# donahowe/TheaterGen

Measured on AMD Instinct MI355X. Metric: 512px 50-step char images/sec (node), CMIGBench 4-turn story, higher is better.
Workload: dtype bf16

## Files before the change

### theatergen_amd/build.py

```python
import hashlib
import os
import subprocess
import sys
from concurrent.futures import ThreadPoolExecutor

HERE = os.path.dirname(os.path.abspath(__file__))
CSRC = os.path.join(HERE, "csrc")
OBJ = os.path.join(CSRC, "_build")
LIBDIR = os.path.join(HERE, "lib")
LIB = os.path.join(LIBDIR, "libtheatergen_hip.so")
HEADER = os.path.join(os.path.dirname(HERE), "include", "theatergen_hip.h")
ARCH = "gfx950"
FLAGS = ["--offload-arch=" + ARCH, "-O3", "-std=c++17", "-fPIC",
         "-Wno-unused-result"]


EXTRA_FLAGS = {"tg_rowchain.hip": ["-mllvm", "-pragma-unroll-threshold=1000000"]}

BUILD_INFO = os.path.join(LIBDIR, "build_info.json")


def _write_build_info():
    import json

    def git(*a):
        try:
            return subprocess.run(["git", "-C", HERE] + list(a), capture_output=True, text=True).stdout.strip()
        except OSError:
            return ""
    info = {"commit": git("rev-parse", "--short", "HEAD"), "csrc_dirty": bool(git("status", "--porcelain", "--", CSRC, HEADER)),
            "sources_sha256": _digest(sources() + sorted(os.path.join(CSRC, f) for f in os.listdir(CSRC) if f.endswith(".h")) + [HEADER])[:16]}
    with open(BUILD_INFO, "w") as f:
        json.dump(info, f)


def _hipcc():
    for c in (os.environ.get("HIPCC"), "/opt/rocm/bin/hipcc", "hipcc"):
        if c and (os.path.isabs(c) and os.path.exists(c) or not os.path.isabs(c)):
            return c
    return "hipcc"


def _digest(paths):
    h = hashlib.sha256()
    for p in paths:
        with open(p, "rb") as f:
            h.update(f.read())
    h.update(" ".join(FLAGS).encode())
    for p_ in paths:
        h.update(" ".join(EXTRA_FLAGS.get(os.path.basename(p_), [])).encode())
    return h.hexdigest()


def sources():
    return sorted(os.path.join(CSRC, f) for f in os.listdir(CSRC) if f.endswith(".hip"))


def build(force=False, verbose=True, check_gate=False):
    os.makedirs(OBJ, exist_ok=True)
    os.makedirs(LIBDIR, exist_ok=True)
    srcs = sources()
    deps = [os.path.join(CSRC, f) for f in os.listdir(CSRC) if f.endswith(".h")] + [HEADER]
    hipcc = _hipcc()
    todo = []
    objs = []
    for s in srcs:
        o = os.path.join(OBJ, os.path.basename(s)[:-4] + ".o")
        stamp = o + ".sha"
        dg = _digest([s] + deps)
        objs.append(o)
        if force or not os.path.exists(o) or not os.path.exists(o + ".res") or not os.path.exists(stamp) or open(stamp).read() != dg:
            todo.append((s, o, stamp, dg))

    def compile_one(job):
        s, o, stamp, dg = job
        cmd = [hipcc] + FLAGS + EXTRA_FLAGS.get(os.path.basename(s), []) + ["-Rpass-analysis=kernel-resource-usage", "-c", s, "-o", o]
        if verbose:
            print("[build]", " ".join(cmd), flush=True)
        r = subprocess.run(cmd, capture_output=True, text=True)
        if r.returncode != 0:
            raise RuntimeError(f"hipcc failed for {s}:\n{r.stdout}\n{r.stderr}")
        with open(o + ".res", "w") as f:
            f.write(r.stderr)
        with open(stamp, "w") as f:
            f.write(dg)

    if todo:
        with ThreadPoolExecutor(max_workers=min(8, len(todo))) as ex:
            list(ex.map(compile_one, todo))
    if todo or not os.path.exists(LIB):
        cmd = [hipcc, "--offload-arch=" + ARCH, "-shared", "-fPIC", "-o", LIB] + objs
        if verbose:
            print("[build]", " ".join(cmd), flush=True)
        r = subprocess.run(cmd, capture_output=True, text=True)
        if r.returncode != 0:
            raise RuntimeError(f"link failed:\n{r.stdout}\n{r.stderr}")
    if todo or not os.path.exists(BUILD_INFO):
        _write_build_info()
    if check_gate or os.environ.get("TG_BUILD_GATE") == "1":
        write_resources(check=True, verbose=verbose, report=False)
    return LIB


RESOURCES_JSON = os.path.join(os.path.dirname(HERE), "profiles", "r6_kernel_resources.json")
HOT_GATES = [
    ("attention_kernel<bf16,48,64,true,true,false,false>", 0, 128),
    ("attention_kernel<f16,48,64,true,true,false,false>", 0, 128),
    ("attention_kernel<", 0, 256),
    ("gemm_glds_kernel<", 0, 256),
    ("conv_halo_kernel<", 0, 256),
    ("conv_slab_kernel<", 320, 256),
    ("bt_gemm_kernel<", 132, 256),
    ("rc_xattn_kernel<", 0, 256),
    ("rc_ff_kernel<", 0, 256),
    ("rc_front_kernel<", 0, 216),
    ("rc_linear_kernel<", 0, 256),
    ("skinny_gemm_kernel<", 0, 256),
    ("attn_bwd_kernel<", 0, 224),
    ("pp_gemm_kernel<bf16,2,", 0, 256),
    ("pp_gemm_kernel<f16,2,", 0, 256),
    ("pp_gemm_kernel<bf16,0,0>", 0, 256),
    ("pp_gemm_kernel<f16,0,0>", 0, 256),
    ("pp_gemm_kernel<", 256, 256),
    ("conv_in_mfma_kernel<", 0, 256),
    ("conv_out_mfma_kernel<", 0, 128),
]


def _pretty(sym):
    import re
    m = re.match(r"_ZN12_GLOBAL__N_1(\d+)", sym) or re.match(r"_Z(\d+)", sym)
    if not m:
        return sym
    n = int(m.group(1))
    base, rest = sym[m.end():m.end() + n], sym[m.end() + n:]
    if not rest.startswith("I"):
        return base
    args, i = [], 1
    while i < len(rest) and rest[i] != "E":
        if rest.startswith("DF16b", i):
            args.append("bf16"); i += 5
        elif rest.startswith("DF16_", i):
            args.append("f16"); i += 5
        elif rest[i] == "L":
            j = rest.index("E", i)
            tok = rest[i + 1:j]
            if tok[0] == "b":
                args.append("true" if tok[1:] == "1" else "false")
            else:
                args.append(re.sub(r"^[a-z]n?", lambda mm: "-" if mm.group(0).endswith("n") and len(mm.group(0)) > 1 else "", tok))
            i = j + 1
        elif rest[i] in "fidjlmb":
            args.append({"f": "float", "i": "int", "d": "double", "j": "unsigned", "l": "long", "m": "unsigned long", "b": "bool"}[rest[i]]); i += 1
        else:
            args.append("?" + rest[i:i + 12]); break
    return base + "<" + ",".join(args) + ">"


def _demangle(names):
    return [_pretty(n) for n in names]


def kernel_resources(verbose=True):
    import re
    keys = {"VGPRs": "vgprs", "AGPRs": "agprs", "ScratchSize [bytes/lane]": "scratch", "Occupancy [waves/SIMD]": "occupancy",
            "SGPRs Spill": "sgpr_spill", "VGPRs Spill": "vgpr_spill", "SGPRs": "sgprs"}
    all_recs = []
    for src in sources():
        path = os.path.join(OBJ, os.path.basename(src)[:-4] + ".o.res")
        if not os.path.exists(path):
            raise RuntimeError(f"{path} is missing: run build() first")
        cur = None
        for line in open(path).read().splitlines():
            m = re.search(r"remark: Function Name: (\S+)", line)
            if m:
                cur = {"symbol": m.group(1), "file": os.path.basename(src)}
                all_recs.append(cur)
                continue
            m = re.search(r"remark:\s+([A-Za-z][A-Za-z \[\]/]*): (\d+)", line)
            if m and cur is not None and m.group(1).strip() in keys:
                cur[keys[m.group(1).strip()]] = int(m.group(2))
    names = _demangle([r["symbol"] for r in all_recs])
    out = {}
    for r, n in zip(all_recs, names):
        r = dict(r)
        if n in out:
            n = n + " " + r["symbol"]
        out[n] = r
    if verbose:
        print(f"[resources] {len(out)} kernels", flush=True)
    return out


def check_resources(res):
    bad = []
    hits = [0] * len(HOT_GATES)
    for name, r in res.items():
        for gi, (sub, max_scratch, max_vgpr) in enumerate(HOT_GATES):
            if sub in name:
                hits[gi] += 1
                if r.get("scratch", 0) > max_scratch or r.get("vgprs", 0) > max_vgpr:
                    bad.append(f"{name}: {r.get('vgprs')} VGPRs (<= {max_vgpr}), scratch {r.get('scratch')} B (<= {max_scratch})")
                break
    for (sub, _, _), n in zip(HOT_GATES, hits):
        if n == 0:
            bad.append(f"gate '{sub}' matches no kernel")
    return bad


ASM_MFMA_KERNELS = {"tg_conv_slab_pp.o": "conv_slab_pp_kernel"}


def check_mfma_loops(verbose=True):
    import re
    import tempfile
    llvm = os.path.join(os.path.dirname(os.path.realpath(_hipcc())), "..", "lib", "llvm", "bin")
    if not os.path.exists(os.path.join(llvm, "llvm-objdump")):
        llvm = "/opt/rocm/lib/llvm/bin"
    bad = []

    def regs(tok):
        m = re.match(r"v\[(\d+):(\d+)\]", tok)
        if m:
            return set(range(int(m.group(1)), int(m.group(2)) + 1))
        m = re.match(r"v(\d+)$", tok)
        return {int(m.group(1))} if m else set()

    for obj, sub in ASM_MFMA_KERNELS.items():
        o = os.path.join(OBJ, obj)
        if not os.path.exists(o):
            continue
        with tempfile.TemporaryDirectory(prefix="tg_isa_") as td:
            fb, co = os.path.join(td, "k.fatbin"), os.path.join(td, "k.co")
            subprocess.run([os.path.join(llvm, "llvm-objcopy"), "--dump-section", ".hip_fatbin=" + fb, o], check=True)
            subprocess.run([os.path.join(llvm, "clang-offload-bundler"), "--unbundle", "--type=o", "--input=" + fb,
                            "--targets=hipv4-amdgcn-amd-amdhsa--" + ARCH, "--output=" + co], check=True)
            dis = subprocess.run([os.path.join(llvm, "llvm-objdump"), "-d", "--no-show-raw-insn", co], capture_output=True, text=True, check=True).stdout
        kern, body, kernels = None, [], []
        for line in dis.split("\n"):
            m = re.match(r"^[0-9a-f]+ <(.*)>:$", line)
            if m:
                if kern is not None:
                    kernels.append((kern, body))
                kern, body = m.group(1), []
            elif kern is not None:
                body.append(line.split("//")[0].strip())
        if kern is not None:
            kernels.append((kern, body))
        seen = 0
        for name, body in kernels:
            if sub not in name:
                continue
            mf = [i for i, t in enumerate(body) if t.startswith("v_mfma")]
            if not mf:
                continue
            seen += 1
            loop = body[mf[0]:mf[-1] + 1]
            accs = set()
            for t in loop:
                if t.startswith("v_mfma"):
                    accs |= regs(t.split(None, 1)[1].split(",")[0].strip())
            hits = [t for t in loop if t and not t.startswith("v_mfma") and any(regs(x) & accs for x in re.findall(r"v\[\d+:\d+\]|v\d+", t))]
            if hits:
                bad.append(f"{_pretty(name)}: {len(hits)} instruction(s) inside the inline-asm MFMA loop touch an accumulator register, e.g. `{hits[0]}`")
        if verbose:
            print(f"[mfma-loops] {obj}: {seen} kernels checked", flush=True)
        if seen == 0:
            bad.append(f"{obj}: no kernel matching {sub!r} with MFMAs found (the check would be vacuous)")
    return bad


def write_resources(check=False, verbose=True, report=True):
    import json
    res = kernel_resources(verbose=verbose)
    if report:
        try:
            commit = subprocess.run(["git", "rev-parse", "--short", "HEAD"], capture_output=True, text=True, cwd=HERE).stdout.strip()
        except OSError:
# ... 23 lines not shown
```

### theatergen_amd/csrc/tg_gemm.hip

```cpp
#include "tg_gemm_common.h"
#include "tg_gemm_glds.h"

namespace {

struct TileCfg { int bm, bn, bk; };
const TileCfg kTiles[] = {{128, 128, 64}, {64, 64, 64}, {128, 64, 64}, {64, 128, 64}, {128, 128, 64}, {256, 256, 64}, {128, 128, 32},
                          {128, 160, 64}, {128, 160, 64}, {128, 160, 64}};
constexpr int kNumTiles = 10;

struct Plan { int tile; bool halo; int full, tail, s, kps; long tiles_m, tiles_n; };



template <typename T>
__global__ void splitk_reduce_kernel(GemmParams p);

inline int64_t plan_workspace_bytes(const Plan& pl) {
  return pl.s > 1 ? (int64_t)pl.tail * pl.s * kTiles[pl.tile].bm * kTiles[pl.tile].bn * 4 : 0;
}

template <typename T>
int launch_reduce(const GemmParams& p, const Plan& pl, hipStream_t st) {
  if (pl.s > 1) {
    hipLaunchKernelGGL(splitk_reduce_kernel<T>, dim3((unsigned)pl.tail * 8), dim3(256), 0, st, p);
    TG_LAUNCH_CHECK();
  }
  return TG_OK;
}

inline bool halo_eligible(const tg_gemm_desc* d) {
  if (d->mode != 1 || d->stride != 1 || d->pad_mode != 0 || d->force_tile != 0 || d->force_split_k > 1 || d->act != TG_ACT_NONE || d->geglu) return false;
  if (d->c0 % BK != 0 || (d->a1 && d->c1 % BK != 0) || d->M % 128 != 0) return false;
  if (d->out_w == 8) return d->out_h == 8 && !d->upsample && d->M >= 1024;
  if (d->out_w != 16 && d->out_w != 32 && d->out_w != 64) return false;
  const int th = 128 / d->out_w;
  if (d->out_h % th != 0) return false;
  return d->M >= 4096;
}

template <typename T>
__global__ __launch_bounds__(256) void splitk_reduce_kernel(GemmParams p) {
  const int t = blockIdx.x >> 3, slice = blockIdx.x & 7;
  const int lbid = p.full_tiles + t;
  const long m0 = (long)(lbid / p.tiles_n) * p.tile_bm, n0 = (long)(lbid % p.tiles_n) * p.tile_bn;
  const int q4 = p.tile_bn / 4;
  const int rows = p.tile_bm / 8;
  const long tile_elems = (long)p.tile_bm * p.tile_bn;
  const float* base = p.ws + (long)t * p.tail_s * tile_elems;
  for (int q = threadIdx.x; q < rows * q4; q += blockDim.x) {
    const int lr = slice * rows + q / q4, lc = (q % q4) * 4;
    f32x4 s = {0.f, 0.f, 0.f, 0.f};
    for (int z = 0; z < p.tail_s; ++z) s += *reinterpret_cast<const f32x4*>(base + z * tile_elems + (long)lr * p.tile_bn + lc);
    const long m = p.patch_pwl > 0 ? patch_token(p, lbid / p.tiles_n, lr) : m0 + lr;
    epilogue_store4<T>(p, m, n0 + lc, s[0], s[1], s[2], s[3]);
  }
}


inline bool halo_eligible(const tg_gemm_desc* d);

inline long t64_max_tiles() {
  const char* e = getenv("TG_T64_MAX");
  return e ? strtol(e, nullptr, 0) : 128;
}

inline int t160_mode() {
  const char* e = getenv("TG_T160");
  return e ? (int)strtol(e, nullptr, 0) : 7;
}

inline long t3_max_tiles() {
  const char* e = getenv("TG_T3_MAX");
  return e ? strtol(e, nullptr, 0) : 256;
}

Plan make_plan(const tg_gemm_desc* d) {
  const long M = d->M, N = d->N, K = d->K;
  const bool halo = halo_eligible(d);
  int t = 0;
  if (!halo) {
    if (N <= 64 && M > 64) t = 2;
    else if (M <= 64 && N > 64) t = 3;
    else if (M <= 64 && N <= 64) t = 1;
    else if (d->mode == 0 && !d->geglu && ((M + 127) / 128) * ((N + 127) / 128) <= t64_max_tiles()) t = 1;
    else if (d->mode == 0 && !d->geglu && N <= 1280 && ((M + 127) / 128) * ((N + 127) / 128) <= t3_max_tiles()) t = 2;
    {
      const char* mk = getenv("TG_T7_MAXK");
      const long maxk = mk ? strtol(mk, nullptr, 0) : 640;
      if (t == 0 && d->mode == 0 && !d->geglu && K <= maxk && K % 32 == 0) t = 6;
      {
        const long t128 = ((M + 127) / 128) * ((N + 127) / 128);
        const char* fit = getenv("TG_T7_FIT");
        if (fit && fit[0] == '1' && t == 0 && d->mode == 0 && !d->geglu && K % 32 == 0 && t128 > 512 && t128 <= 768) t = 6;
      }
    }
    if ((t == 0 || t == 6) && d->mode == 0 && !d->geglu && d->act == TG_ACT_NONE && d->n_split <= 0 && N % 160 == 0 && M % 128 == 0 && K % 64 == 0 && (t160_mode() & 5)) {
      const long t128 = ((M + 127) / 128) * ((N + 127) / 128), s128 = (t == 6) ? 768 : 512;
      const long t160 = (M / 128) * (N / 160);
      const double eff128 = (double)t128 / (double)(((t128 + s128 - 1) / s128) * s128);
      const double e256 = (double)t160 / (double)(((t160 + 255) / 256) * 256), e512 = (double)t160 / (double)(((t160 + 511) / 512) * 512);
      const bool one_per_cu = e256 > e512 + 1e-9;
      const double eff160 = one_per_cu ? e256 : e512;
      const bool ragged128 = N % 128 != 0 && K >= 640 && (t160_mode() & 4);
      if (d->force_split_k <= 1 && t160 >= 192 && (((t160_mode() & 1) && eff160 >= eff128 + 0.1) || (ragged128 && eff160 >= eff128 - 0.01))) t = one_per_cu ? 7 : 9;
    }
    if (d->force_tile >= 21 && d->force_tile <= 23) t = d->force_tile - 14;
    else if (d->force_tile > 0) t = d->force_tile - 1;
    if (t >= kNumTiles || t < 0) t = 0;
  }
  const long tm = (M + kTiles[t].bm - 1) / kTiles[t].bm, tn = (N + kTiles[t].bn - 1) / kTiles[t].bn;
  const long T = tm * tn;
  const int units = halo ? (int)((d->c0 + (d->a1 ? d->c1 : 0)) / BK) : (int)((K + kTiles[t].bk - 1) / kTiles[t].bk);
  const int min_units = halo ? 2 : 8;
  long S = 512;
  if (!halo && (t == 1 || t == 6)) S = 768;
  if (!halo && (t == 4 || t == 5 || t == 7)) S = 256;
  long full = (T / S) * S, rem = T - full;
  int s = 1;
  if (d->force_split_k > 0) {
    full = 0; rem = T; s = d->force_split_k;
  } else if (rem > 0 && !d->geglu && units >= 2 * min_units) {
    const double t_unit = halo ? 9.0 : (d->mode == 1 ? 1.5 : 1.1), t_fix = 6.0;
    const double unsplit = (units * t_unit + t_fix) * (2 * rem <= S ? ((!halo && d->mode == 1) ? 0.85 : 0.6) : 1.0);
    double best = 1e30;
    int best_c = 1;
    for (int c = 2; c <= 8 && units / c >= min_units; ++c) {
      const int kps = (units + c - 1) / c;
      const long rounds = (rem * c + S - 1) / S;
      const double cost = rounds * (kps * t_unit + t_fix) + 6.0 + 0.065 * (double)(rem * c);
      if (cost < best) { best = cost; best_c = c; }
    }
    if (best < unsplit * 0.95) s = best_c;
  }
  if (s > units) s = units;
  if (s < 1) s = 1;
  int kps = (units + s - 1) / s;
  s = (units + kps - 1) / kps;
  if (s <= 1) { s = 1; full = T; rem = 0; kps = units; }
  return Plan{t, halo, (int)full, (int)rem, s, kps, tm, tn};
}

template <typename T, int BM, int BN, int WM, int WN, bool CONV, int STAGES, int BKT, int EPI>
void launch_glds(const GemmParams& p, dim3 grid, size_t lds, hipStream_t st) {
  auto k = gemm_glds_kernel<T, BM, BN, WM, WN, CONV, STAGES, BKT, EPI>;
  static const hipError_t attr = hipFuncSetAttribute(reinterpret_cast<const void*>(k), hipFuncAttributeMaxDynamicSharedMemorySize, (int)lds);
  (void)attr;
  hipLaunchKernelGGL(k, grid, dim3(WM * WN * 64), lds, st, p);
}

template <typename T, int BM, int BN, int WM, int WN, int STAGES, int BKT = 64>
int launch_cfg2(const tg_gemm_desc* d, const GemmParams& p, const Plan& pl, hipStream_t st) {
  const size_t lds = (size_t)STAGES * (BM + BN) * BKT * sizeof(T);
  dim3 grid((unsigned)(pl.full + pl.tail * pl.s));
  constexpr bool kMainTile = (BM == 128 && BN == 128 && STAGES == 2) || (BM == 256 && BN == 256);
  const int epi = d->geglu ? ((kMainTile && d->mode != 1) ? 2 : 1) : (d->act == TG_ACT_NONE ? 0 : 1);
  if (d->mode == 1) {
    if (epi == 0) launch_glds<T, BM, BN, WM, WN, true, STAGES, BKT, 0>(p, grid, lds, st);
    else launch_glds<T, BM, BN, WM, WN, true, STAGES, BKT, 1>(p, grid, lds, st);
  } else {
    if (epi == 0) launch_glds<T, BM, BN, WM, WN, false, STAGES, BKT, 0>(p, grid, lds, st);
    else if (epi == 2) {
      if constexpr (kMainTile) launch_glds<T, BM, BN, WM, WN, false, STAGES, BKT, 2>(p, grid, lds, st);
    } else launch_glds<T, BM, BN, WM, WN, false, STAGES, BKT, 1>(p, grid, lds, st);
  }
  TG_LAUNCH_CHECK();
  return launch_reduce<T>(p, pl, st);
}

}
int tg_gemm_bt_launch(const tg_gemm_desc* d, const void* params, int bt_tile, void* stream);
int tg_conv_slab_launch(const tg_gemm_desc* d, const void* params, int splits, void* stream);
bool tg_conv_slab_is_pp(const tg_gemm_desc* d, int patch_pwl, int patch_np, int epi_lds);
int tg_gemm_ln_launch(const tg_gemm_desc* d, const void* params, int short_k, int grid, void* stream);
int tg_gemm_t160_launch(const tg_gemm_desc* d, const void* params, int variant, int grid, void* stream);
int tg_conv_halo_launch(const tg_gemm_desc* d, const void* params, int grid, void* stream);
int tg_gemm_pp_launch(const tg_gemm_desc* d, const void* params, void* stream);
int tg_gemm_pp160_launch(const tg_gemm_desc* d, const void* params, void* stream);
namespace {

inline bool slab_geometry(const tg_gemm_desc* d, int* pw, int* np, bool* patch) {
  const int w = d->out_w, h = d->out_h;
  int P = 0, NPv = 1;
  if (w == 64 || w == 32 || w == 16) P = w;
  else if (w % 64 == 0) P = 64;
  else if (w % 32 == 0) P = 32;
  else if (w % 16 == 0) P = 16;
  else if (w % 8 == 0) { P = 8; NPv = 2; }
  else return false;
  const int th = 128 / (P * NPv);
  if (h % th != 0 || d->M % 128 != 0) return false;
  *pw = P; *np = NPv; *patch = (P != w) || NPv > 1;
  return true;
}

inline int slab_splits_of(const tg_gemm_desc* d) {
  if (d->mode != 1 || d->stride != 1 || d->upsample || d->pad_mode != 0 || d->act != TG_ACT_NONE || d->geglu) return 0;
  if (d->N % 320 != 0 || d->c0 % BK != 0 || (d->a1 && d->c1 % BK != 0) || d->n_split > 0) return 0;
  int pw, np;
  bool patch;
  if (!slab_geometry(d, &pw, &np, &patch)) return 0;
  const int chunks = (d->c0 + (d->a1 ? d->c1 : 0)) / BK;
  if (d->force_tile == 11) {
    if (d->force_split_k <= 1) return 1;
    if (d->force_split_k > chunks) return 0;
    const int cps = (chunks + d->force_split_k - 1) / d->force_split_k;
    return (chunks + cps - 1) / cps;
  }
  if (d->force_split_k > 1) return 0;
  if (d->force_tile == 12) return chunks >= 2 ? 2 : 0;
  if (d->force_tile != 0) return 0;
  long flags = 0;
  { const char* e = getenv("TG_GEMM_FLAGS"); flags = e ? strtol(e, nullptr, 0) : 0; }
  const bool old_patch = (d->out_w == 128 || d->out_w == 96);
  if ((flags & 128) || (old_patch && (flags & 1024))) return 0;
  const long t = (d->M / 128) * (d->N / 320);
  auto full = [](long n) { return 4 * n >= 3 * ((n + 255) / 256) * 256; };
  if (!patch || old_patch) {
    if (old_patch && t >= 128) return 1;
    if (!old_patch && full(t)) return 1;
    if (!old_patch && chunks >= 10 && full(2 * t)) return 2;
  }
  if (flags & 2048) return 0;
  if (halo_eligible(d) && !(flags & 4096)) return 0;
  const double t_red = 8.0, t_part = 0.02;
  double best = 1e30;
  int best_s = 0;
  for (int c = 1; c <= 8; ++c) {
    const int cps = (chunks + c - 1) / c;
    if (c > 1 && (cps < 2 || (chunks + cps - 1) / cps != c)) continue;
    const long items = t * c;
    const long rounds = (items + 255) / 256;
    const double per_round = (double)(items < 256 ? items : 256);
    const double t_k = per_round / 210.0 > 0.9 ? per_round / 210.0 : 0.9;
    const double cost = rounds * 9.0 * cps * t_k + (c > 1 ? t_red + t_part * (double)items : 0.0);
    if (cost < best) { best = cost; best_s = c; }
  }
  if (t * best_s < 96) return 0;
  return best_s;
}

inline int bt_tile_of(const tg_gemm_desc* d) {
  const int ft = d->force_tile;
  const bool can = d->mode == 0 && d->force_split_k <= 1 && d->a1 == nullptr && d->K % BK == 0;
  if (ft == 10) return can ? 2 : -1;
  if (ft == 9) return -1;
  if (ft != 0 || !can) return -1;
  int devf = 0;
  { const char* e = getenv("TG_GEMM_FLAGS"); devf = e ? (int)strtol(e, nullptr, 0) : 0; }
  if (devf & 8) return -1;
  if (d->geglu) {
    const long tiles = ((d->M + 255) / 256) * ((d->N + 255) / 256);
    return (d->M >= 16384 && tiles >= 1024) ? 2 : -1;
  }
  return -1;
}

inline int pp_mode() {
  const char* e = getenv("TG_PP");
  return e ? (int)strtol(e, nullptr, 0) : 15;
}
inline bool pp_eligible(const tg_gemm_desc* d) {
  if (d->mode != 0 || d->a1 != nullptr || d->force_split_k > 1 || d->a_coef != nullptr) return false;
  if (d->M % 256 != 0 || d->N % 256 != 0 || d->K % 64 != 0 || d->K < 128) return false;
  if (d->n_split > 0 && (d->n_split % 64 != 0 || d->rows_per_batch <= 0 || (d->M / d->rows_per_batch) * (d->N - d->n_split) * d->ldt >= (1LL << 31))) return false;
  if (d->ln_u != nullptr && d->ln_rows == nullptr) return false;
  if (d->geglu && d->n_split > 0) return false;
  auto al16 = [](const void* q) { return (reinterpret_cast<uintptr_t>(q) & 15) == 0; };
  const long lda = d->lda > 0 ? d->lda : d->c0, ldw = d->ldw > 0 ? d->ldw : d->K;
  if (!(al16(d->a0) && al16(d->w) && al16(d->out) && al16(d->bias) && al16(d->bvec) && al16(d->res)) || lda % 8 != 0 || ldw % 8 != 0 || d->ldc % 8 != 0) return false;
  if ((d->bvec != nullptr && d->ldbvec % 8 != 0) || (d->res != nullptr && d->ldres % 8 != 0)) return false;
  if (d->a_rows_per_batch > 0 && d->a_batch_stride % 8 != 0) return false;
  return true;
}
inline bool pp_selected(const tg_gemm_desc* d) {
  if (d->force_tile == 24) return pp_eligible(d);
  if (d->force_tile != 0 || !pp_eligible(d)) return false;
  const int mode = pp_mode();
  if (d->ln_u != nullptr ? !(mode & 4) : (d->geglu ? !(mode & 1) : !(mode & 2))) return false;
  const long tiles = (d->M / 256) * (d->N / 256);
  const double eff = (double)tiles / (double)(((tiles + 255) / 256) * 256);
  return tiles >= 192 && eff >= 0.6 && d->K >= 640;
}

inline bool pp160_eligible(const tg_gemm_desc* d) {
  if (d->mode != 0 || d->a1 != nullptr || d->force_split_k > 1 || d->a_coef != nullptr || d->geglu) return false;
  if (d->M % 256 != 0 || d->N % 160 != 0 || d->K % 64 != 0 || d->K < 128) return false;
  if (d->n_split > 0 && (d->n_split % 80 != 0 || d->rows_per_batch <= 0 || (d->M / d->rows_per_batch) * (d->N - d->n_split) * d->ldt >= (1LL << 31))) return false;
  if (d->ln_u != nullptr && d->ln_rows == nullptr) return false;
  auto al16 = [](const void* q) { return (reinterpret_cast<uintptr_t>(q) & 15) == 0; };
  const long lda = d->lda > 0 ? d->lda : d->c0, ldw = d->ldw > 0 ? d->ldw : d->K;
  if (!(al16(d->a0) && al16(d->w) && al16(d->out) && al16(d->bias) && al16(d->bvec) && al16(d->res)) || lda % 8 != 0 || ldw % 8 != 0 || d->ldc % 8 != 0) return false;
  if ((d->bvec != nullptr && d->ldbvec % 8 != 0) || (d->res != nullptr && d->ldres % 8 != 0)) return false;
  if (d->a_rows_per_batch > 0 && d->a_batch_stride % 8 != 0) return false;
  return true;
}
inline bool pp160_selected(const tg_gemm_desc* d) {
  if (d->force_tile == 25) return pp160_eligible(d);
  if (d->force_tile != 0 || !pp160_eligible(d) || !(pp_mode() & 8)) return false;
  if (d->ln_u != nullptr && !(pp_mode() & 4)) return false;
  const long tiles = (d->M / 256) * (d->N / 160);
  const double eff = (double)tiles / (double)(((tiles + 255) / 256) * 256);
  return tiles >= 192 && eff >= 0.74 && d->K >= 640;
}

inline int ln_t160_of(const tg_gemm_desc* d) {
  if (!(t160_mode() & 2) || d->geglu || d->N % 160 != 0 || d->M % 128 != 0 || d->K % 64 != 0 || d->n_split > 0) return 0;
  const long t128 = (d->M / 128) * ((d->N + 127) / 128), s128 = d->K <= 640 ? 768 : 512;
  const long t160 = (d->M / 128) * (d->N / 160);
  const double eff128 = (double)t128 / (double)(((t128 + s128 - 1) / s128) * s128);
  const double e256 = (double)t160 / (double)(((t160 + 255) / 256) * 256), e512 = (double)t160 / (double)(((t160 + 511) / 512) * 512);
  const bool one_per_cu = e256 > e512 + 1e-9;
  const double eff160 = one_per_cu ? e256 : e512;
  if (t160 < 192 || eff160 < eff128 + 0.05) return 0;
  return one_per_cu ? 160 : 161;
}

inline bool epi_lds_of(const tg_gemm_desc* d) {
  auto al16 = [](const void* q) { return (reinterpret_cast<uintptr_t>(q) & 15) == 0; };
  return d->N % 8 == 0 && d->ldc % 8 == 0 && al16(d->out) && al16(d->bias) && al16(d->bvec) && al16(d->res) &&
         (d->bvec == nullptr || d->ldbvec % 8 == 0) && (d->res == nullptr || d->ldres % 8 == 0) && (d->n_split == 0 || d->n_split % 64 == 0);
}

inline int gn_partial_blocks_of(const tg_gemm_desc* d) {
  if (d->out_gn_groups <= 0 || d->N % d->out_gn_groups != 0 || 80 % (d->N / d->out_gn_groups) != 0) return 0;
  if (slab_splits_of(d) != 1) return 0;
  int pw = 0, np = 1;
  bool patch = false;
  if (!slab_geometry(d, &pw, &np, &patch) || patch || np != 1) return 0;
  if (!tg_conv_slab_is_pp(d, 0, 1, epi_lds_of(d))) return 0;
  const long hw = (long)d->out_h * d->out_w;
  if (hw % 64 != 0) return 0;
  return (int)(hw / 64);
}

template <typename T>
int launch_gemm(const tg_gemm_desc* d, hipStream_t st) {
  Plan pl = make_plan(d);
  GemmParams p{};
  p.a0 = d->a0; p.a1 = d->a1; p.c0 = d->c0; p.c1 = d->a1 ? d->c1 : 0;
  p.in_h = d->in_h; p.in_w = d->in_w; p.out_h = d->out_h; p.out_w = d->out_w;
  p.stride = d->stride; p.upsample = d->upsample; p.pad_lo = d->pad_mode == 1 ? 0 : 1;
  p.w = d->w; p.M = d->M; p.N = d->N; p.K = d->K;
  p.bias = d->bias; p.bvec = d->bvec; p.ldbvec = d->ldbvec;
  p.rows_per_batch = d->rows_per_batch > 0 ? d->rows_per_batch : d->M;
  p.res = d->res; p.ldres = d->ldres; p.act = d->act; p.geglu = d->geglu; p.out_scale = d->out_scale;
  p.out = d->out; p.ldc = d->ldc; p.n_split = d->n_split; p.out_t = d->out_t; p.ldt = d->ldt;
  p.ws = reinterpret_cast<float*>(d->workspace);
  p.full_tiles = pl.full; p.tail_s = pl.s; p.kt_per_split = pl.kps; p.tiles_n = (int)pl.tiles_n;
  p.tile_bm = kTiles[pl.tile].bm; p.tile_bn = kTiles[pl.tile].bn;
  p.a_rpb = d->mode == 0 ? d->a_rows_per_batch : 0; p.a_bs = d->a_batch_stride;
  p.lda = d->lda > 0 ? d->lda : p.c0; p.ldw = d->ldw > 0 ? d->ldw : d->K;
  {
    const char* e = getenv("TG_GEMM_FLAGS");
    p.flags = e ? (int)strtol(e, nullptr, 0) : 0;
  }
  p.a_coef = d->a_coef; p.a_silu = d->a_silu;
  p.patch_pwl = 0; p.patch_np = 1;
  p.ln_u = d->ln_u; p.ln_v = d->ln_v; p.ln_eps = d->ln_eps; p.ln_rows = d->ln_rows;
  p.epi_lds = epi_lds_of(d);
  p.gn_part = d->out_gn_partials; p.gn_cpg = d->out_gn_partials ? (int)(d->N / d->out_gn_groups) : 0;
  TG_CHECK(d->out_gn_partials == nullptr || gn_partial_blocks_of(d) > 0, TG_ERR_UNSUPPORTED,
           "tg_gemm: out_gn_partials needs an unsplit stride-1 conv on the two-wave slab kernel with 80 %% (N / groups) == 0 (ask tg_gemm_gn_partial_blocks)");
  if (pp_selected(d)) return tg_gemm_pp_launch(d, &p, st);
  if (pp160_selected(d)) return tg_gemm_pp160_launch(d, &p, st);
  TG_CHECK(d->force_tile != 25, TG_ERR_UNSUPPORTED, "tg_gemm: force_tile 25 (ping-pong 256 x 160 tiles) needs a plain single-source GEMM with M %% 256 == 0, N %% 160 == 0, K %% 64 == 0, 16-byte aligned operands and no GEGLU");
  TG_CHECK(d->force_tile != 24, TG_ERR_UNSUPPORTED, "tg_gemm: force_tile 24 (ping-pong 256 x 256 tiles) needs a plain single-source GEMM with M %% 256 == 0, N %% 256 == 0, K %% 64 == 0 and 16-byte aligned operands");
  if (d->ln_u != nullptr) {
    const int t160 = ln_t160_of(d);
    const int bn = t160 ? 160 : 128;
    const long tiles = ((d->M + 127) / 128) * ((d->N + bn - 1) / bn);
    p.full_tiles = (int)tiles; p.tail_s = 1; p.tiles_n = (int)((d->N + bn - 1) / bn); p.tile_bm = 128; p.tile_bn = bn;
    p.kt_per_split = 0;
    return tg_gemm_ln_launch(d, &p, t160 ? t160 : (d->K <= 640 ? 1 : 0), (int)tiles, st);
  }
  if (const int sp = slab_splits_of(d); sp > 0) {
    const long tiles = (d->M / 128) * (d->N / 320);
    if (sp > 1) {
      const int64_t need = tiles * sp * 128 * 320 * 4;
      TG_CHECK(d->workspace != nullptr && d->workspace_bytes >= need, TG_ERR_ARG, "tg_gemm conv: the K split needs %lld workspace bytes, got %lld",
               (long long)need, (long long)d->workspace_bytes);
    }
    {
      int pw = 0, np = 1;
      bool patch = false;
      slab_geometry(d, &pw, &np, &patch);
      p.patch_np = np;
      if (patch) { int l = 0; while ((1 << l) < pw) ++l; p.patch_pwl = l; }
    }
    int rc = tg_conv_slab_launch(d, &p, sp, st);
    if (rc != TG_OK || sp == 1) return rc;
    p.tiles_n = (int)(d->N / 320); p.full_tiles = 0; p.tail_s = sp; p.tile_bm = 128; p.tile_bn = 320;
    Plan rp = pl;
    rp.tail = (int)tiles; rp.s = sp;
    return launch_reduce<T>(p, rp, st);
  }
  TG_CHECK(d->a_coef == nullptr, TG_ERR_UNSUPPORTED, "tg_gemm: a_coef (GroupNorm prologue) needs a problem the slab conv kernel takes (tg_gemm_plan kernel_kind 4)");
  {
    const int64_t need = plan_workspace_bytes(pl);
    TG_CHECK(need == 0 || (d->workspace != nullptr && d->workspace_bytes >= need), TG_ERR_ARG,
             "tg_gemm: the K-split tail needs %lld workspace bytes, got %lld", (long long)need, (long long)d->workspace_bytes);
  }
  if (const int bt = bt_tile_of(d); bt >= 0) {
    TG_CHECK(d->lda <= 0 && d->ldw <= 0, TG_ERR_UNSUPPORTED, "tg_gemm: lda / ldw are taken by the 128 x 128 / 128 x 160 plain kernels only");
    TG_CHECK(!d->geglu || bt == 2, TG_ERR_ARG, "tg_gemm: the GEGLU epilogue needs the 256 x 256 big tile (force_tile 10)");
    TG_CHECK(d->n_split <= 0 || d->n_split % 128 == 0, TG_ERR_ARG, "tg_gemm: the big tile needs n_split on a wave-tile boundary");
    return tg_gemm_bt_launch(d, &p, bt, st);
  }
  if (pl.halo) {
    const int rc = tg_conv_halo_launch(d, &p, pl.full + pl.tail * pl.s, st);
    if (rc != TG_OK) return rc;
    return launch_reduce<T>(p, pl, st);
  }
  switch (pl.tile) {
    case 0: return launch_cfg2<T, 128, 128, 2, 2, 2>(d, p, pl, st);
    case 1: return launch_cfg2<T, 64, 64, 2, 2, 3>(d, p, pl, st);
    case 2: return launch_cfg2<T, 128, 64, 4, 1, 3>(d, p, pl, st);
    case 3: return launch_cfg2<T, 64, 128, 1, 4, 3>(d, p, pl, st);
    case 4: return launch_cfg2<T, 128, 128, 2, 2, 3>(d, p, pl, st);
    case 6: return launch_cfg2<T, 128, 128, 2, 2, 3, 32>(d, p, pl, st);
    case 7: case 8: case 9: {
      TG_CHECK(d->mode == 0 && !d->geglu && d->act == TG_ACT_NONE, TG_ERR_ARG, "tg_gemm: the 128 x 160 tiles take plain GEMMs with a linear epilogue");
      const int rc = tg_gemm_t160_launch(d, &p, pl.tile - 7, pl.full + pl.tail * pl.s, st);
      if (rc != TG_OK) return rc;
      return launch_reduce<T>(p, pl, st);
    }
    default: return launch_cfg2<T, 256, 256, 2, 4, 2>(d, p, pl, st);
  }
}

int validate(const tg_gemm_desc* d) {
  TG_CHECK(d != nullptr, TG_ERR_ARG, "tg_gemm: null descriptor");
  TG_CHECK(d->dtype == TG_BF16 || d->dtype == TG_F16, TG_ERR_ARG, "tg_gemm: bad dtype %d", d->dtype);
  TG_CHECK(d->a0 && d->w && d->out, TG_ERR_ARG, "tg_gemm: null a0/w/out");
  TG_CHECK((reinterpret_cast<uintptr_t>(d->a0) & 15) == 0 && (reinterpret_cast<uintptr_t>(d->a1) & 15) == 0 && (reinterpret_cast<uintptr_t>(d->w) & 15) == 0,
           TG_ERR_ARG, "tg_gemm: a0 / a1 / w must be 16-byte aligned (a0=%p a1=%p w=%p)", d->a0, d->a1, d->w);
  TG_CHECK(d->M > 0 && d->N > 0 && d->K > 0, TG_ERR_ARG, "tg_gemm: empty problem M=%lld N=%lld K=%lld",
           (long long)d->M, (long long)d->N, (long long)d->K);
  TG_CHECK(d->N % 4 == 0 && d->K % 8 == 0, TG_ERR_ARG, "tg_gemm: N %% 4 and K %% 8 required (N=%lld K=%lld)",
           (long long)d->N, (long long)d->K);
  if (d->geglu) {
    TG_CHECK(d->N % 64 == 0 && d->n_split <= 0 && !d->bvec && !d->res && d->act == TG_ACT_NONE && d->force_split_k <= 1,
             TG_ERR_ARG, "tg_gemm: GEGLU epilogue needs N %% 64 == 0 (packed a|gate groups) and no other epilogue terms");
    const int ft = d->force_tile;
    TG_CHECK(ft == 0 || ft == 1 || ft == 5 || ft == 6 || ft == 10 || ft == 24, TG_ERR_ARG, "tg_gemm: GEGLU epilogue needs a tile with 64-column wave tiles");
    TG_CHECK(d->M > 64, TG_ERR_ARG, "tg_gemm: GEGLU epilogue needs M > 64");
  }
  const int ctot = d->c0 + (d->a1 ? d->c1 : 0);
  if (d->a1) TG_CHECK(d->c0 % BK == 0, TG_ERR_ARG, "tg_gemm: two-source A needs c0 %% 64 == 0 (c0=%d)", d->c0);
  TG_CHECK(d->a_coef == nullptr || d->mode == 1, TG_ERR_ARG, "tg_gemm: a_coef is a conv (mode 1) argument");
  if (d->mode == 1) {
    TG_CHECK(ctot % BK == 0, TG_ERR_ARG, "tg_gemm conv: channels %% 64 required (c=%d)", ctot);
    TG_CHECK(d->K == 9L * ctot, TG_ERR_ARG, "tg_gemm conv: K must be 9*(c0+c1)");
    TG_CHECK(d->stride == 1 || d->stride == 2, TG_ERR_ARG, "tg_gemm conv: stride 1|2");
    TG_CHECK(!(d->upsample && d->stride != 1), TG_ERR_ARG, "tg_gemm conv: upsample needs stride 1");
    TG_CHECK(d->M == (int64_t)d->batch * d->out_h * d->out_w, TG_ERR_ARG, "tg_gemm conv: M != batch*out_h*out_w");
    TG_CHECK(d->pad_mode == 0 || (d->pad_mode == 1 && d->stride == 2 && !d->upsample), TG_ERR_ARG,
             "tg_gemm conv: pad_mode 1 (bottom / right padding) is the stride-2 encoder downsample only");
    const int pad2 = d->pad_mode == 1 ? 1 : 2;
    const int eh = d->upsample ? 2 * d->in_h : (d->in_h + pad2 - 3) / d->stride + 1;
    const int ew = d->upsample ? 2 * d->in_w : (d->in_w + pad2 - 3) / d->stride + 1;
    TG_CHECK(eh == d->out_h && ew == d->out_w, TG_ERR_ARG, "tg_gemm conv: out %dx%d inconsistent with in %dx%d",
             d->out_h, d->out_w, d->in_h, d->in_w);
  } else {
    TG_CHECK(d->mode == 0, TG_ERR_ARG, "tg_gemm: bad mode %d", d->mode);
    TG_CHECK(ctot == d->K, TG_ERR_ARG, "tg_gemm: K (%lld) != c0+c1 (%d)", (long long)d->K, ctot);
    if (d->a_rows_per_batch > 0)
      TG_CHECK(d->a1 == nullptr && d->a_batch_stride % 8 == 0, TG_ERR_ARG, "tg_gemm: batched A needs a single source and a 16-byte aligned batch pitch");
  }
  if (d->n_split > 0) {
    TG_CHECK(d->out_t && d->n_split % 4 == 0 && d->rows_per_batch > 0, TG_ERR_ARG, "tg_gemm: bad transposed-output args");
  }
  if (d->lda > 0 || d->ldw > 0) {
    TG_CHECK(d->mode == 0 && d->a1 == nullptr && d->a_rows_per_batch <= 0 && d->ln_u == nullptr, TG_ERR_ARG,
             "tg_gemm: lda / ldw belong to the plain single-source GEMM (no conv, no second source, no batched A, no LayerNorm fold)");
    TG_CHECK((d->lda <= 0 || (d->lda >= d->K && d->lda % 8 == 0)) && (d->ldw <= 0 || (d->ldw >= d->K && d->ldw % 8 == 0)), TG_ERR_ARG,
             "tg_gemm: lda = %lld / ldw = %lld must be >= K and multiples of 8", (long long)d->lda, (long long)d->ldw);
  }
// ... 75 lines not shown
```

### theatergen_amd/csrc/tg_norm.hip

```cpp
#include "tg_common.h"

namespace {

constexpr int GN_MAX_CHUNKS = 4;

struct GnParams {
  const void* x0;
  const void* x1;
  int c0, c1;
  int batch;
  long hw;
  int groups;
  float eps;
  const void* gamma;
  const void* beta;
  int silu;
  void* out;
  float* partials;
  float* stats;
  int nblk;
  int npart;
  int cx, ry;
  float* coef;
};

template <typename T>
__device__ __forceinline__ typename Vec<T>::v8 gn_load8(const GnParams& p, int b, long pix, int ch) {
  typedef typename Vec<T>::v8 V8;
  if (ch < p.c0) return *reinterpret_cast<const V8*>(reinterpret_cast<const T*>(p.x0) + ((long)b * p.hw + pix) * p.c0 + ch);
  return *reinterpret_cast<const V8*>(reinterpret_cast<const T*>(p.x1) + ((long)b * p.hw + pix) * p.c1 + (ch - p.c0));
}

template <typename T>
__global__ __launch_bounds__(256) void gn_partial_kernel(GnParams p) {
  extern __shared__ float sh[];
  const int C = p.c0 + p.c1;
  const int cpr = C / 8;
  const int b = blockIdx.y;
  const int blk = blockIdx.x;
  const long per = (p.hw + p.nblk - 1) / p.nblk;
  const long p_begin = (long)blk * per;
  long p_end = p_begin + per;
  if (p_end > p.hw) p_end = p.hw;
  const int tx = threadIdx.x % p.cx;
  const int ty = threadIdx.x / p.cx;
  if (ty < p.ry) {
    float* mine = sh + (size_t)ty * 2 * C;
    for (int c = tx; c < cpr; c += p.cx) {
      float s[8], q[8];
#pragma unroll
      for (int j = 0; j < 8; ++j) { s[j] = 0.f; q[j] = 0.f; }
      long pix = p_begin + ty;
      for (; pix + 3 * (long)p.ry < p_end; pix += 4 * (long)p.ry) {
        typename Vec<T>::v8 v0 = gn_load8<T>(p, b, pix, c * 8);
        typename Vec<T>::v8 v1 = gn_load8<T>(p, b, pix + p.ry, c * 8);
        typename Vec<T>::v8 v2 = gn_load8<T>(p, b, pix + 2 * (long)p.ry, c * 8);
        typename Vec<T>::v8 v3 = gn_load8<T>(p, b, pix + 3 * (long)p.ry, c * 8);
#pragma unroll
        for (int j = 0; j < 8; ++j) {
          const float f0 = to_f32<T>(v0[j]), f1 = to_f32<T>(v1[j]), f2 = to_f32<T>(v2[j]), f3 = to_f32<T>(v3[j]);
          s[j] += f0; q[j] += f0 * f0;
          s[j] += f1; q[j] += f1 * f1;
          s[j] += f2; q[j] += f2 * f2;
          s[j] += f3; q[j] += f3 * f3;
        }
      }
      for (; pix < p_end; pix += p.ry) {
        typename Vec<T>::v8 v = gn_load8<T>(p, b, pix, c * 8);
#pragma unroll
        for (int j = 0; j < 8; ++j) {
          float f = to_f32<T>(v[j]);
          s[j] += f;
          q[j] += f * f;
        }
      }
#pragma unroll
      for (int j = 0; j < 8; ++j) {
        mine[c * 8 + j] = s[j];
        mine[C + c * 8 + j] = q[j];
      }
    }
  }
  __syncthreads();
  for (int i = threadIdx.x; i < 2 * C; i += blockDim.x) {
    float a = sh[i];
    for (int r = 1; r < p.ry; ++r) a += sh[(size_t)r * 2 * C + i];
    sh[i] = a;
  }
  __syncthreads();
  const int cpg = C / p.groups;
  for (int g = threadIdx.x; g < p.groups; g += blockDim.x) {
    float s = 0.f, q = 0.f;
    for (int j = 0; j < cpg; ++j) { s += sh[g * cpg + j]; q += sh[C + g * cpg + j]; }
    float* o = p.partials + (((long)b * p.nblk + blk) * p.groups + g) * 2;
    o[0] = s;
    o[1] = q;
  }
}

__device__ __forceinline__ void gn_block_stats(const GnParams& p, int b, float* s_stats ) {
  __shared__ double sh[8][32][2];
  const int C = p.c0 + p.c1;
  const double cnt = (double)p.hw * (C / p.groups);
  const int part = threadIdx.x >> 5, gl = threadIdx.x & 31;
  for (int g0 = 0; g0 < p.groups; g0 += 32) {
    const int g = g0 + gl;
    double s = 0.0, q = 0.0;
    if (g < p.groups)
      for (int k = part; k < p.npart; k += 8) {
        const float* o = p.partials + (((long)b * p.npart + k) * p.groups + g) * 2;
        s += (double)o[0];
        q += (double)o[1];
      }
    sh[part][gl][0] = s;
    sh[part][gl][1] = q;
    __syncthreads();
    if (part == 0 && g < p.groups) {
      for (int r = 1; r < 8; ++r) { s += sh[r][gl][0]; q += sh[r][gl][1]; }
      const double mean = s / cnt;
      double var = q / cnt - mean * mean;
      if (var < 0.0) var = 0.0;
      s_stats[g * 2] = (float)mean;
      s_stats[g * 2 + 1] = (float)(1.0 / sqrt(var + (double)p.eps));
    }
    __syncthreads();
  }
}

template <typename T>
__global__ __launch_bounds__(256) void gn_apply_kernel(GnParams p) {
  typedef typename Vec<T>::v8 V8;
  const int C = p.c0 + p.c1;
  const int cpr = C / 8;
  const int cpg = C / p.groups;
  const int b = blockIdx.y;
  const int blk = blockIdx.x;
  const long per = (p.hw + p.nblk - 1) / p.nblk;
  const long p_begin = (long)blk * per;
  long p_end = p_begin + per;
  if (p_end > p.hw) p_end = p.hw;
  extern __shared__ float s_stats[];
  const int tx = threadIdx.x % p.cx;
  const int ty = threadIdx.x / p.cx;
  V8 pre0, pre1, pre2, pre3;
  const bool have_pre = ty < p.ry && tx < cpr && p_begin + ty + 3 * (long)p.ry < p_end;
  if (have_pre) {
    const long pix = p_begin + ty;
    pre0 = gn_load8<T>(p, b, pix, tx * 8);
    pre1 = gn_load8<T>(p, b, pix + p.ry, tx * 8);
    pre2 = gn_load8<T>(p, b, pix + 2 * (long)p.ry, tx * 8);
    pre3 = gn_load8<T>(p, b, pix + 3 * (long)p.ry, tx * 8);
  }
  gn_block_stats(p, b, s_stats);
  if (ty >= p.ry) return;
  const T* gam = reinterpret_cast<const T*>(p.gamma);
  const T* bet = reinterpret_cast<const T*>(p.beta);
  T* out = reinterpret_cast<T*>(p.out);
  for (int c = tx; c < cpr; c += p.cx) {
    float a[8], d[8];
#pragma unroll
    for (int j = 0; j < 8; ++j) {
      const int ch = c * 8 + j;
      const int g = ch / cpg;
      const float mean = s_stats[g * 2];
      const float rstd = s_stats[g * 2 + 1];
      const float ga = gam ? to_f32<T>(gam[ch]) : 1.f;
      const float be = bet ? to_f32<T>(bet[ch]) : 0.f;
      a[j] = rstd * ga;
      d[j] = be - mean * a[j];
    }
    auto norm8 = [&](const V8& v) {
      V8 o;
#pragma unroll
      for (int j = 0; j < 8; ++j) {
        float f = to_f32<T>(v[j]) * a[j] + d[j];
        if (p.silu) f = silu_f(f);
        o[j] = from_f32<T>(f);
      }
      return o;
    };
    long pix = p_begin + ty;
    if (c == tx && have_pre) {
      T* o0 = out + ((long)b * p.hw + pix) * C + c * 8;
      *reinterpret_cast<V8*>(o0) = norm8(pre0);
      *reinterpret_cast<V8*>(o0 + (long)p.ry * C) = norm8(pre1);
      *reinterpret_cast<V8*>(o0 + 2 * (long)p.ry * C) = norm8(pre2);
      *reinterpret_cast<V8*>(o0 + 3 * (long)p.ry * C) = norm8(pre3);
      pix += 4 * (long)p.ry;
    }
    for (; pix + 3 * (long)p.ry < p_end; pix += 4 * (long)p.ry) {
      const V8 v0 = gn_load8<T>(p, b, pix, c * 8);
      const V8 v1 = gn_load8<T>(p, b, pix + p.ry, c * 8);
      const V8 v2 = gn_load8<T>(p, b, pix + 2 * (long)p.ry, c * 8);
      const V8 v3 = gn_load8<T>(p, b, pix + 3 * (long)p.ry, c * 8);
      T* o0 = out + ((long)b * p.hw + pix) * C + c * 8;
      *reinterpret_cast<V8*>(o0) = norm8(v0);
      *reinterpret_cast<V8*>(o0 + (long)p.ry * C) = norm8(v1);
      *reinterpret_cast<V8*>(o0 + 2 * (long)p.ry * C) = norm8(v2);
      *reinterpret_cast<V8*>(o0 + 3 * (long)p.ry * C) = norm8(v3);
    }
    for (; pix < p_end; pix += p.ry) {
      const V8 v = gn_load8<T>(p, b, pix, c * 8);
      *reinterpret_cast<V8*>(out + ((long)b * p.hw + pix) * C + c * 8) = norm8(v);
    }
  }
}

template <typename T>
__global__ __launch_bounds__(256) void gn_coef_kernel(GnParams p) {
  __shared__ float s_stats[2 * 256];
  const int C = p.c0 + p.c1;
  const int cpg = C / p.groups;
  const int b = blockIdx.x;
  gn_block_stats(p, b, s_stats);
  const T* gam = reinterpret_cast<const T*>(p.gamma);
  const T* bet = reinterpret_cast<const T*>(p.beta);
  float* ca = p.coef + (long)b * 2 * C;
  for (int ch = threadIdx.x; ch < C; ch += blockDim.x) {
    const int g = ch / cpg;
    const float mean = s_stats[g * 2];
    const float rstd = s_stats[g * 2 + 1];
    const float ga = gam ? to_f32<T>(gam[ch]) : 1.f;
    const float be = bet ? to_f32<T>(bet[ch]) : 0.f;
    const float a = rstd * ga;
    ca[ch] = a;
    ca[C + ch] = be - mean * a;
  }
}

template <typename T, int MAXP>
__global__ __launch_bounds__(256) void gn_small_kernel(GnParams p, int gpb, int nc, int npy) {
  typedef typename Vec<T>::v8 V8;
  __shared__ float red[256];
  __shared__ float col[256];
  __shared__ float gstat[32];
  const int C = p.c0 + p.c1;
  const int cpg = C / p.groups;
  const int ccg = cpg / 8;
  const int b = blockIdx.y;
  const int c = threadIdx.x % nc, py = threadIdx.x / nc;
  const bool active = py < npy;
  const int ch0 = blockIdx.x * gpb * cpg + c * 8;
  const int hw = (int)p.hw;
  V8 v[MAXP];
  V8 gv, bv;
  const T* gam = reinterpret_cast<const T*>(p.gamma);
  const T* bet = reinterpret_cast<const T*>(p.beta);
  if (active) {
    if (gam) gv = *reinterpret_cast<const V8*>(gam + ch0);
    if (bet) bv = *reinterpret_cast<const V8*>(bet + ch0);
  }
  float s = 0.f;
  if (active) {
#pragma unroll
    for (int i = 0; i < MAXP; ++i) {
      const int pix = py + i * npy;
      v[i] = gn_load8<T>(p, b, pix < hw ? pix : hw - 1, ch0);
    }
#pragma unroll
    for (int i = 0; i < MAXP; ++i) {
      if (py + i * npy < hw) {
#pragma unroll
        for (int j = 0; j < 8; ++j) s += to_f32<T>(v[i][j]);
      }
    }
    red[py * nc + c] = s;
  }
  __syncthreads();
  const float inv_n = 1.f / ((float)hw * (float)cpg);
  if ((int)threadIdx.x < nc) {
    float t = 0.f;
    for (int y = 0; y < npy; ++y) t += red[y * nc + threadIdx.x];
    col[threadIdx.x] = t;
  }
  __syncthreads();
  if ((int)threadIdx.x < gpb) {
    float t = 0.f;
    for (int k = 0; k < ccg; ++k) t += col[threadIdx.x * ccg + k];
    gstat[threadIdx.x] = t * inv_n;
  }
  __syncthreads();
  const float mean = active ? gstat[c / ccg] : 0.f;
  float q = 0.f;
  if (active) {
#pragma unroll
    for (int i = 0; i < MAXP; ++i) {
      const int pix = py + i * npy;
      if (pix < hw) {
#pragma unroll
        for (int j = 0; j < 8; ++j) {
          const float d = to_f32<T>(v[i][j]) - mean;
          q += d * d;
        }
      }
    }
    red[py * nc + c] = q;
  }
  __syncthreads();
  if ((int)threadIdx.x < nc) {
    float t = 0.f;
    for (int y = 0; y < npy; ++y) t += red[y * nc + threadIdx.x];
    col[threadIdx.x] = t;
  }
  __syncthreads();
  if ((int)threadIdx.x < gpb) {
    float t = 0.f;
    for (int k = 0; k < ccg; ++k) t += col[threadIdx.x * ccg + k];
    gstat[16 + threadIdx.x] = rsqrtf(t * inv_n + p.eps);
  }
  __syncthreads();
  if (!active) return;
  const float rstd = gstat[16 + c / ccg];
  float a[8], d[8];
#pragma unroll
  for (int j = 0; j < 8; ++j) {
    const float ga = gam ? to_f32<T>(gv[j]) : 1.f;
    const float be = bet ? to_f32<T>(bv[j]) : 0.f;
    a[j] = rstd * ga;
    d[j] = be - mean * a[j];
  }
  if (p.coef != nullptr) {
    if (py == 0) {
      float* ca = p.coef + (long)b * 2 * C + ch0;
#pragma unroll
      for (int j = 0; j < 8; ++j) { ca[j] = a[j]; ca[C + j] = d[j]; }
    }
    return;
  }
  T* out = reinterpret_cast<T*>(p.out);
#pragma unroll
  for (int i = 0; i < MAXP; ++i) {
    const int pix = py + i * npy;
    if (pix < hw) {
      V8 o;
#pragma unroll
      for (int j = 0; j < 8; ++j) {
        float f = to_f32<T>(v[i][j]) * a[j] + d[j];
        if (p.silu) f = silu_f(f);
        o[j] = from_f32<T>(f);
      }
      *reinterpret_cast<V8*>(out + ((long)b * hw + pix) * C + ch0) = o;
    }
  }
}

bool gn_small_plan(int C, int groups, long hw, int* gpb, int* nc, int* npy, int* maxp) {
  const int cpg = C / groups;
  if (hw > 256 || cpg % 8 != 0) return false;
  int g = 1;
  while (g < groups && (g * cpg < 64 || groups % g != 0)) ++g;
  if (groups % g != 0 || g > 16) return false;
  const int n = g * cpg / 8;
  if (n > 256) return false;
  const int y = 256 / n;
  const int mp = (int)((hw + y - 1) / y);
  if (mp > 24) return false;
  *gpb = g; *nc = n; *npy = y; *maxp = mp;
  return true;
}

int gn_nblk(int batch, long hw) {
  long target = 512 / (batch > 0 ? batch : 1);
  if (target < 1) target = 1;
  long nblk = hw / 8;
  if (nblk > target) nblk = target;
  if (nblk < 1) nblk = 1;
  return (int)nblk;
}

template <typename T, int LPR, int MAXC>
__global__ __launch_bounds__(256) void layernorm_kernel(const T* x, long rows, int C, long ldx, float eps, const T* gamma,
                                                        const T* beta, T* out, long ldo, float* stats = nullptr) {
  typedef typename Vec<T>::v8 V8;
  constexpr int RPW = 64 / LPR;
  const int lane = threadIdx.x & 63;
  const int l = lane % LPR;
  const long row = ((long)blockIdx.x * 4 + (threadIdx.x >> 6)) * RPW + lane / LPR;
  const bool row_ok = row < rows;
  const int cpr = C / 8;
// ... 199 lines not shown
```

Baseline: 9.385.

## Flatten split-K reduce, batch GN partial loads, prefetch GN coefficients

```diff
diff --git a/theatergen_amd/build.py b/theatergen_amd/build.py
--- a/theatergen_amd/build.py
+++ b/theatergen_amd/build.py
@@ -124,6 +124,8 @@
     ("pp_gemm_kernel<", 256, 256),
     ("conv_in_mfma_kernel<", 0, 256),
     ("conv_out_mfma_kernel<", 0, 128),
+    ("conv_slab_pp_kernel<", 108, 168),
+    ("pp160_gemm_kernel<", 0, 256),
 ]
 
 
diff --git a/theatergen_amd/csrc/tg_gemm.hip b/theatergen_amd/csrc/tg_gemm.hip
--- a/theatergen_amd/csrc/tg_gemm.hip
+++ b/theatergen_amd/csrc/tg_gemm.hip
@@ -12,17 +12,34 @@
 
 
 
-template <typename T>
+template <typename T, int S>
 __global__ void splitk_reduce_kernel(GemmParams p);
 
 inline int64_t plan_workspace_bytes(const Plan& pl) {
   return pl.s > 1 ? (int64_t)pl.tail * pl.s * kTiles[pl.tile].bm * kTiles[pl.tile].bn * 4 : 0;
+}
+
+inline bool reduce_flat() {
+  static const int v = [] { const char* e = getenv("TG_REDUCE_FLAT"); return e ? (int)strtol(e, nullptr, 0) : 1; }();
+  return v != 0;
 }
 
 template <typename T>
 int launch_reduce(const GemmParams& p, const Plan& pl, hipStream_t st) {
   if (pl.s > 1) {
-    hipLaunchKernelGGL(splitk_reduce_kernel<T>, dim3((unsigned)pl.tail * 8), dim3(256), 0, st, p);
+    const unsigned per_tile = (unsigned)((long)p.tile_bm * p.tile_bn / 4 / 256);
+    const dim3 flat((unsigned)pl.tail * per_tile);
+#define TG_REDUCE(SS) hipLaunchKernelGGL((splitk_reduce_kernel<T, SS>), flat, dim3(256), 0, st, p)
+    if (!reduce_flat() || pl.s > 8 || (long)per_tile * 256 * 4 != (long)p.tile_bm * p.tile_bn)
+      hipLaunchKernelGGL((splitk_reduce_kernel<T, 0>), dim3((unsigned)pl.tail * 8), dim3(256), 0, st, p);
+    else if (pl.s == 2) TG_REDUCE(2);
+    else if (pl.s == 3) TG_REDUCE(3);
+    else if (pl.s == 4) TG_REDUCE(4);
+    else if (pl.s == 5) TG_REDUCE(5);
+    else if (pl.s == 6) TG_REDUCE(6);
+    else if (pl.s == 7) TG_REDUCE(7);
+    else TG_REDUCE(8);
+#undef TG_REDUCE
     TG_LAUNCH_CHECK();
   }
   return TG_OK;
@@ -38,8 +55,27 @@
   return d->M >= 4096;
 }
 
-template <typename T>
+template <typename T, int S>
 __global__ __launch_bounds__(256) void splitk_reduce_kernel(GemmParams p) {
+  if constexpr (S > 0) {
+    const long tile_elems = (long)p.tile_bm * p.tile_bn;
+    const int per_tile = (int)(tile_elems / 4 / 256);
+    const int t = blockIdx.x / per_tile;
+    const int q = (blockIdx.x - t * per_tile) * 256 + (int)threadIdx.x;
+    const int q4 = p.tile_bn / 4;
+    const int lr = q / q4, lc = (q - lr * q4) * 4;
+    const int lbid = p.full_tiles + t;
+    const float* src = p.ws + (long)t * S * tile_elems + (long)lr * p.tile_bn + lc;
+    f32x4 v[S];
+#pragma unroll
+    for (int z = 0; z < S; ++z) v[z] = *reinterpret_cast<const f32x4*>(src + z * tile_elems);
+    f32x4 s = {0.f, 0.f, 0.f, 0.f};
+#pragma unroll
+    for (int z = 0; z < S; ++z) s += v[z];
+    const long m = p.patch_pwl > 0 ? patch_token(p, lbid / p.tiles_n, lr) : (long)(lbid / p.tiles_n) * p.tile_bm + lr;
+    epilogue_store4<T>(p, m, (long)(lbid % p.tiles_n) * p.tile_bn + lc, s[0], s[1], s[2], s[3]);
+    return;
+  }
   const int t = blockIdx.x >> 3, slice = blockIdx.x & 7;
   const int lbid = p.full_tiles + t;
   const long m0 = (long)(lbid / p.tiles_n) * p.tile_bm, n0 = (long)(lbid % p.tiles_n) * p.tile_bn;
@@ -322,7 +358,7 @@
 }
 
 inline int gn_partial_blocks_of(const tg_gemm_desc* d) {
-  if (d->out_gn_groups <= 0 || d->N % d->out_gn_groups != 0 || 80 % (d->N / d->out_gn_groups) != 0) return 0;
+  if (d->out_gn_groups <= 0 || d->N % d->out_gn_groups != 0 || 80 % (d->N / d->out_gn_groups) != 0 || (d->N / d->out_gn_groups) % 2 != 0) return 0;
   if (slab_splits_of(d) != 1) return 0;
   int pw = 0, np = 1;
   bool patch = false;
diff --git a/theatergen_amd/csrc/tg_norm.hip b/theatergen_amd/csrc/tg_norm.hip
--- a/theatergen_amd/csrc/tg_norm.hip
+++ b/theatergen_amd/csrc/tg_norm.hip
@@ -107,10 +107,19 @@
     const int g = g0 + gl;
     double s = 0.0, q = 0.0;
     if (g < p.groups)
-      for (int k = part; k < p.npart; k += 8) {
-        const float* o = p.partials + (((long)b * p.npart + k) * p.groups + g) * 2;
-        s += (double)o[0];
-        q += (double)o[1];
+      for (int k0 = part; k0 < p.npart; k0 += 64) {
+        float2 v[8];
+#pragma unroll
+        for (int u = 0; u < 8; ++u) {
+          const int k = k0 + 8 * u < p.npart ? k0 + 8 * u : k0;
+          v[u] = *reinterpret_cast<const float2*>(p.partials + (((long)b * p.npart + k) * p.groups + g) * 2);
+        }
+#pragma unroll
+        for (int u = 0; u < 8; ++u)
+          if (k0 + 8 * u < p.npart) {
+            s += (double)v[u].x;
+            q += (double)v[u].y;
+          }
       }
     sh[part][gl][0] = s;
     sh[part][gl][1] = q;
@@ -212,19 +221,38 @@
   const int C = p.c0 + p.c1;
   const int cpg = C / p.groups;
   const int b = blockIdx.x;
-  gn_block_stats(p, b, s_stats);
+  constexpr int GN_COEF_CPT = 8;
   const T* gam = reinterpret_cast<const T*>(p.gamma);
   const T* bet = reinterpret_cast<const T*>(p.beta);
+  float ga[GN_COEF_CPT], be[GN_COEF_CPT];
+#pragma unroll
+  for (int u = 0; u < GN_COEF_CPT; ++u) {
+    const int ch = (int)threadIdx.x + u * (int)blockDim.x;
+    const int cl = ch < C ? ch : C - 1;
+    ga[u] = gam ? to_f32<T>(gam[cl]) : 1.f;
+    be[u] = bet ? to_f32<T>(bet[cl]) : 0.f;
+  }
+  gn_block_stats(p, b, s_stats);
   float* ca = p.coef + (long)b * 2 * C;
-  for (int ch = threadIdx.x; ch < C; ch += blockDim.x) {
+#pragma unroll
+  for (int u = 0; u < GN_COEF_CPT; ++u) {
+    const int ch = (int)threadIdx.x + u * (int)blockDim.x;
+    if (ch < C) {
+      const int g = ch / cpg;
+      const float a = s_stats[g * 2 + 1] * ga[u];
+      ca[ch] = a;
+      ca[C + ch] = be[u] - s_stats[g * 2] * a;
+    }
+  }
+  for (int ch = threadIdx.x + GN_COEF_CPT * blockDim.x; ch < C; ch += blockDim.x) {
     const int g = ch / cpg;
     const float mean = s_stats[g * 2];
     const float rstd = s_stats[g * 2 + 1];
-    const float ga = gam ? to_f32<T>(gam[ch]) : 1.f;
-    const float be = bet ? to_f32<T>(bet[ch]) : 0.f;
-    const float a = rstd * ga;
+    const float ga1 = gam ? to_f32<T>(gam[ch]) : 1.f;
+    const float be1 = bet ? to_f32<T>(bet[ch]) : 0.f;
+    const float a = rstd * ga1;
     ca[ch] = a;
-    ca[C + ch] = be - mean * a;
+    ca[C + ch] = be1 - mean * a;
   }
 }
 
```

After: 9.429 (median of 6 runs). No clear change (+0.5%).
